# ahoynodnarb/minidiff

Measured on AMD Instinct MI355X. Metric: forward+backward passes/sec on 4096x4096 fp32 matmul+elementwise graph, higher is better.
Workload: dtype f32

## Files before the change

minidiff_amd/csrc/gemm.hip:

```cpp
#include <stdlib.h>

#include <algorithm>
#include <type_traits>
#include <utility>
#include <vector>

#include <hip/hip_ext.h>

#include "md_hip.h"

extern "C" int mdhip_alloc(size_t, void **);
extern "C" int mdhip_unary(int, const mdhip_array *, const mdhip_array *);
extern "C" int mdhip_free(void *);
extern "C" int mdhip_convert(const mdhip_array *, const mdhip_array *);

namespace {

typedef float f32x16 __attribute__((ext_vector_type(16)));
typedef float f32x4 __attribute__((ext_vector_type(4)));

constexpr int LDP = 4;

struct GemmArgs {
  const float *A, *B;
// ... 943 lines not shown
      if (s < 2) {
#pragma unroll
        for (int q = 0; q < 2; ++q) {
          glds64_krow(A, g.a_ks, kn * BK, CUR ? A0 : A1, (2 * s + q) * 4 + wave, lo);
          glds64_krow(B, g.b_ks, kn * BK, CUR ? B0 : B1, (2 * s + q) * 4 + wave, lo);
        }
      }
#pragma unroll
      for (int i = 0; i < WTM; ++i)
#pragma unroll
        for (int j = 0; j < WTN; ++j) acc[i][j] = __builtin_amdgcn_mfma_f64_16x16x4f64(fa[c][i], fb[c][j], acc[i][j], 0, 0, 0);
#pragma unroll
      for (int m = 0; m < WTM * WTN; ++m) {
        __builtin_amdgcn_sched_group_barrier(0x008, 1, 0);
        if (m < 8 && s + 1 < 4) __builtin_amdgcn_sched_group_barrier(0x100, 1, 0);
        if (s < 2 && m < 4) __builtin_amdgcn_sched_group_barrier(0x010, 1, 0);
      }
    }
    __syncthreads();
    MD_F64_READ(CUR ^ 1, 0, 0)
  };
  MD_KTILE_ROTATE(2, nk, ktile)
#undef MD_F64_READ
  MD_STORE_C64(false, acc, C, g, m0, n0, wm, wn, l16, h)
}


static const float *md_zero_block() {
  static const float *z = [] {
    void *p = nullptr;
    if (hipMalloc(&p, 64) != hipSuccess || hipMemset(p, 0, 64) != hipSuccess) return (const float *)nullptr;
    return (const float *)p;
  }();
  return z;
}

static bool md_gemm_nbuf3(int64_t blocks, int64_t K, int bk) {
  if (K < 2 * bk) return false;
  if (const int64_t f = md_opt(MD_OPT_GEMM_NBUF)) return f == 3;
  return blocks <= MD_NUM_CUS;
}

static void md_gemm_launch(void (*kernel)(GemmArgs), dim3 grid, int threads, const GemmArgs &ga) {
  hipEvent_t e0, e1;
  if (md_prof_take(&e0, &e1)) hipExtLaunchKernelGGL(kernel, grid, dim3((unsigned)threads), 0, md_stream(), e0, e1, 0, ga);
  else hipLaunchKernelGGL(kernel, grid, dim3((unsigned)threads), 0, md_stream(), ga);
}

struct StampDump {
  static constexpr size_t kMax = 8192;
  unsigned long long *dev = nullptr;
  int bm = 0, bn = 0, bk = 0;
  size_t blocks = 0;
  static StampDump &get() { static StampDump d; return d; }
  unsigned long long *buffer() {
    if (!dev) (void)hipMalloc((void **)&dev, kMax * 16);
    return dev;
  }
  void note(int m, int n, int k, size_t b) { bm = m; bn = n; bk = k; blocks = b; }
  ~StampDump() {
    if (!dev || !blocks) return;
    std::vector<unsigned long long> h(blocks * 2);
    if (hipDeviceSynchronize() != hipSuccess || hipMemcpy(h.data(), dev, h.size() * 8, hipMemcpyDeviceToHost) != hipSuccess) return;
    std::vector<double> ghz, us;
    for (size_t b = 0; b < blocks; ++b)
      if (h[2 * b + 1]) { ghz.push_back((double)h[2 * b] / (double)h[2 * b + 1] * 0.1); us.push_back((double)h[2 * b + 1] * 0.01); }
    std::sort(ghz.begin(), ghz.end());
    std::sort(us.begin(), us.end());
    if (!ghz.empty())
      fprintf(stderr, "[mdhip] last gemm %dx%dx%d: in-kernel clock median %.3f GHz (min %.3f, max %.3f) over %zu blocks; block main loop median %.1f us (min %.1f, p10 %.1f, p90 %.1f, max %.1f)\n",
              bm, bn, bk, ghz[ghz.size() / 2], ghz.front(), ghz.back(), ghz.size(), us[us.size() / 2], us.front(), us[us.size() / 10], us[us.size() * 9 / 10], us.back());
  }
};

enum { CFG_128x128x16 = 0, CFG_64x64x16, CFG_128x64x16, CFG_256x128x16, CFG_256x256x32, CFG_128x128x32, CFG_128x64x32, CFG_128x128_W8, CFG_COUNT };
struct Tile { int bm, bn, bk, wm, wn; };
struct TileCfg { Tile reg[2], dma[2]; double tf[2], tf_dma[2]; };
constexpr TileCfg kTiles[CFG_COUNT] = {
     {{{128, 128, 16, 2, 2}, {128, 128, 16, 2, 2}}, {{128, 128, 32, 2, 2}, {}}, {133.0, 0.0}, {143.0, 0.0}},
     {{{64, 64, 16, 2, 2}, {64, 64, 16, 2, 2}}, {{}, {}}, {120.0, 120.0}, {0.0, 0.0}},
     {{{128, 64, 16, 2, 2}, {128, 64, 16, 2, 2}}, {{}, {}}, {126.0, 0.0}, {0.0, 0.0}},
     {{{256, 128, 16, 2, 2}, {256, 128, 16, 2, 2}}, {{}, {}}, {139.0, 138.0}, {0.0, 0.0}},
     {{{256, 128, 16, 2, 2}, {256, 256, 32, 2, 2}}, {{256, 256, 32, 2, 2}, {256, 256, 32, 2, 2}}, {0.0, 140.0}, {149.0, 150.0}},
     {{{128, 128, 16, 2, 2}, {128, 128, 32, 2, 2}}, {{128, 128, 32, 2, 2}, {128, 128, 32, 2, 2}}, {0.0, 132.0}, {0.0, 146.0}},
     {{{128, 64, 16, 2, 2}, {128, 64, 32, 2, 2}}, {{}, {128, 64, 32, 2, 2}}, {0.0, 126.7}, {0.0, 138.0}},
     {{{128, 128, 16, 2, 4}, {128, 128, 32, 2, 4}}, {{128, 128, 32, 2, 4}, {128, 128, 32, 2, 4}}, {133.0, 134.0}, {143.5, 146.0}},
};
constexpr int kPickOrder[] = {CFG_256x256x32, CFG_256x128x16, CFG_128x128x16, CFG_128x128x32, CFG_128x128_W8, CFG_128x64x16, CFG_128x64x32, CFG_64x64x16};
constexpr bool lds3_fits(Tile t) { return 3 * (t.bm + t.bn) * t.bk * 4 <= 128 * 1024; }

static int pick_cfg(int64_t M, int64_t N, int64_t K, int64_t batch, bool tn, bool dma_ok, double *est = nullptr) {
  if (est) *est = 64.0 * 64.0 / 120.0;
  {
    const int64_t v = md_opt(MD_OPT_GEMM_CFG);
    if (v >= 0 && v < CFG_COUNT) return (int)v;
  }
  if (((M + 63) / 64) * ((N + 63) / 64) * batch < MD_NUM_CUS && K >= 1024) return CFG_64x64x16;
  int best = CFG_64x64x16;
  double best_t = 1e300;
  for (const int cfg : kPickOrder) {
    const TileCfg &c = kTiles[cfg];
    const bool dma = dma_ok && c.tf_dma[tn] > 0.0;
    const double tf = dma ? c.tf_dma[tn] : c.tf[tn];
    if (tf <= 0.0) continue;
    const Tile t = dma ? c.dma[tn] : c.reg[tn];
    const int64_t tiles = ((M + t.bm - 1) / t.bm) * ((N + t.bn - 1) / t.bn) * batch;
    double s = (double)((tiles + MD_NUM_CUS - 1) / MD_NUM_CUS) * t.bm * t.bn / tf;
    if (tiles <= MD_NUM_CUS && cfg != CFG_128x128_W8 && cfg != CFG_256x256x32 && !(tn && dma && cfg == CFG_128x128x32)) s /= 0.8;
    if (cfg == CFG_256x256x32 && tiles < MD_NUM_CUS) continue;
    if (!dma && ((M % t.bm) || (N % t.bn) || (K % 16))) s /= 0.85;
    if (s < best_t * 0.999) { best_t = s; best = cfg; }
  }
  if (est && best_t < 1e299) *est = best_t;
  return best;
}

template <class GA> static bool dma_family(const GA &ga, bool a_kc, bool b_kc) {
  return md_opt(MD_OPT_GEMM_GLDS) != 0 && (a_kc ? ga.a_ks == 1 : ga.a_ms == 1) && (b_kc ? ga.b_ks == 1 : ga.b_ns == 1) && (a_kc || !b_kc);
}
static bool dma_pieces_whole(const GemmArgs &ga, bool a_kc, bool b_kc) {
  return ((a_kc || b_kc) ? ga.K % 4 == 0 : true) && (a_kc || ga.M % 4 == 0 || ga.pad_m) && (b_kc || ga.N % 4 == 0 || ga.pad_n);
}
constexpr int64_t kLane32 = 1ll << 26;
template <class GA> static bool dma_strides(const GA &ga, bool a_kc, bool b_kc, int64_t lim) {
// ... 386 lines not shown
  constexpr bool TN = !A_KC && !B_KC;
  constexpr Tile R = kTiles[CFG].reg[TN], D = kTiles[CFG].dma[TN];
  constexpr int SCHED = R.bm == 64 ? 0 : 1;
  if (s.staging != ST_REG) {
    if constexpr (D.bm != 0 && A_KC) return kc_kernel<D.bm, D.bn, D.bk, D.wm, D.wn, B_KC>(s);
    else if constexpr (D.bm != 0 && TN) return tn_kernel<D.bm, D.bn, D.bk, D.wm, D.wn>(s);
    else return nullptr;
  }
  if (s.splits > 1) {
    if constexpr (R.bm == 64 && R.bn == 64) return s.edge ? k_gemm_f32_mfma<64, 64, 16, 2, 2, A_KC, B_KC, true, true> : k_gemm_f32_mfma<64, 64, 16, 2, 2, A_KC, B_KC, false, true>;
    else return nullptr;
  }
  if (s.epi) { if constexpr (A_KC && !B_KC) return k_gemm_f32_mfma<R.bm, R.bn, R.bk, R.wm, R.wn, true, false, false, false, SCHED, 1>; else return nullptr; }
  return s.edge ? k_gemm_f32_mfma<R.bm, R.bn, R.bk, R.wm, R.wn, A_KC, B_KC, true> : k_gemm_f32_mfma<R.bm, R.bn, R.bk, R.wm, R.wn, A_KC, B_KC, false, false, SCHED>;
}
template <bool A_KC, bool B_KC, int... C> static GemmKernel f32_kernel(const GemmStep &s, std::integer_sequence<int, C...>) {
  GemmKernel k = nullptr;
  ((s.cfg == C ? (void)(k = cfg_kernel<C, A_KC, B_KC>(s)) : (void)0), ...);
  return k;
}
static GemmKernel f32_kernel(const GemmStep &s) {
  return with_layout(s.a_kc, s.b_kc, [&](auto a, auto b) { return f32_kernel<decltype(a)::value, decltype(b)::value>(s, std::make_integer_sequence<int, CFG_COUNT>{}); });
}
static int run_step(const GemmStep &s, const void *const *tmp, int *skip) {
  auto at = [&](auto q) {
    const uintptr_t u = (uintptr_t)q;
    return (u >> 56) ? (decltype(q))((char *)tmp[(u >> 56) - 1] + (u & ((1ull << 56) - 1))) : q;
  };
  MdGemm g = s.g;
  g.a = at(g.a); g.b = at(g.b); g.c = at(g.c);
  switch (s.kind) {
    case S_LONGK:
    case S_SKINNY: {
      const int rc = s.kind == S_LONGK ? md_gemm_longk(g, s.dtype) : md_gemm_skinny(g, s.dtype);
      *skip = rc < 0 ? 0 : s.skip;
      return rc < 0 ? MDHIP_OK : rc;
    }
    case S_REPACK: {
      if (g.M <= 65535 * 4) {
        k_repack_rows<<<dim3((unsigned)((g.N + 1023) / 1024), (unsigned)((g.M + 3) / 4)), 256, 0, md_stream()>>>((const float *)g.a, g.M, g.N, g.a_ms, (float *)g.c, g.c_ms);
        return MD_LAUNCH_CHECK(s.what);
      }
      mdhip_array sd{}, dd{};
      sd.data = const_cast<void *>(g.a); sd.dtype = MDHIP_F32; sd.ndim = 2; sd.shape[0] = g.M; sd.shape[1] = g.N; sd.strides[0] = g.a_ms; sd.strides[1] = 1;
      dd = sd; dd.data = g.c; dd.strides[0] = g.c_ms;
      return mdhip_unary(MDHIP_U_COPY, &sd, &dd);
    }
    case S_F32: {
      GemmArgs ga = s.ga;
      ga.A = at(ga.A); ga.B = at(ga.B); ga.C = at(ga.C); ga.partial = at(ga.partial); ga.run_if_set = at(ga.run_if_set);
      if (s.epi) ga.tickets = md_tickets();
      const GemmKernel k = f32_kernel(s);
      if (!k) return md_fail(MDHIP_ERUNTIME, "matmul: no kernel for the planned launch (cfg %d)", s.cfg);
      if (s.stamp) ga.stamp = StampDump::get().buffer();
      if (s.stamp) StampDump::get().note(s.tile.bm, s.tile.bn, s.tile.bk, (size_t)s.grid.x * s.grid.z);
      if (s.splits > 1) hipLaunchKernelGGL(k, s.grid, dim3(64u * s.tile.wm * s.tile.wn), 0, md_stream(), ga);
      else md_gemm_launch(k, s.grid, 64 * s.tile.wm * s.tile.wn, ga);
      return MD_LAUNCH_CHECK(s.what);
    }
    case S_SUM:
      k_gemm_splitk_sum<<<md_grid_for(g.batch * g.M * g.N), MD_BLOCK, 0, md_stream()>>>((const float *)g.a, (int)g.K, g.batch, g.M, g.N, (float *)g.c,
                                                                                         g.c_bs, g.c_ms, g.c_ns);
      return MD_LAUNCH_CHECK(s.what);
    case S_F64: {
      auto k = with_layout(s.a_kc, s.b_kc, [&](auto a, auto b) -> void (*)(GemmArgs64) {
        constexpr bool A = decltype(a)::value, B = decltype(b)::value;
        if (s.cfg == 1) return s.edge ? k_gemm_f64_mfma<128, 128, 16, 2, 2, A, B, true> : k_gemm_f64_mfma<128, 128, 16, 2, 2, A, B, false>;
        return s.edge ? k_gemm_f64_mfma<64, 64, 16, 2, 2, A, B, true> : k_gemm_f64_mfma<64, 64, 16, 2, 2, A, B, false>;
      });
      hipLaunchKernelGGL(s.cfg == 2 ? k_gemm_f64_tn_glds : k, s.grid, dim3(256), 0, md_stream(), s.ga64);
      return MD_LAUNCH_CHECK(s.cfg == 2 ? "matmul(f64 mfma, direct-to-LDS)" : s.what);
    }
    case S_NMFMA: {
      const void *zero = s.edge ? md_zero_block() : nullptr;
      if (s.edge && !zero) return md_fail(MDHIP_EMEMORY, "matmul: zero block");
      return s.wide ? md_gemm_widen_mfma(g, s.dtype, s.a_kc, s.b_kc, s.edge, zero) : md_gemm_narrow_mfma(g, s.dtype, s.a_kc, s.b_kc, s.edge, zero);
    }
    case S_BX_CLEAR: return md_hip_check(hipMemsetAsync(const_cast<void *>(g.b), 0, 4, md_stream()), s.what);
    case S_BX_SPLIT_ROWS:
    case S_BX_SPLIT_COLS:
      return md_gemm_bf16x3_split((const float *)g.a, s.kind == S_BX_SPLIT_ROWS, g.M, g.K, g.a_ms, g.c, (unsigned *)const_cast<void *>(g.b), s.cfg,
                                  s.splits == 6 ? 3 : s.splits == 3 ? 2 : 1);
    case S_BX_GEMM:
      return md_gemm_bf16x3(g.a, at(s.b_planes), (float *)g.c, g.M, g.N, g.K, g.c_ms, (const unsigned *)g.b, (int)md_opt(MD_OPT_GEMM_BF16X3_LOOP), s.cfg,
                            (int)md_opt(MD_OPT_GEMM_BF16X3_BAND), s.splits);
    case S_NGENERIC: return s.wide ? md_gemm_widen_generic(g, s.dtype) : md_gemm_narrow_generic(g, s.dtype);
    case S_NCONV: {
      mdhip_array sd{}, dd{};
      sd.data = const_cast<void *>(g.a); sd.dtype = s.dtype; sd.ndim = 3;
      sd.shape[0] = g.batch; sd.shape[1] = g.M; sd.shape[2] = g.N;
      sd.strides[0] = g.a_bs; sd.strides[1] = g.a_ms; sd.strides[2] = g.a_ks;
      dd = sd; dd.data = g.c; dd.dtype = s.dtype_to;
      dd.strides[0] = g.c_bs; dd.strides[1] = g.c_ms; dd.strides[2] = g.c_ns;
      return mdhip_convert(&sd, &dd);
    }
    case S_GENERIC: {
      const dim3 grid((unsigned)((g.N + 15) / 16), (unsigned)((g.M + 15) / 16), (unsigned)g.batch);
      if (grid.y > 65535) return md_fail(MDHIP_EVALUE, "matmul: M too large for the generic kernel");
      switch (s.dtype) {
        case MDHIP_F32: k_gemm_generic<float><<<grid, 256, 0, md_stream()>>>(g); break;
        case MDHIP_F64: k_gemm_generic<double><<<grid, 256, 0, md_stream()>>>(g); break;
        case MDHIP_I32: k_gemm_generic<int32_t><<<grid, 256, 0, md_stream()>>>(g); break;
        default: k_gemm_generic<int64_t><<<grid, 256, 0, md_stream()>>>(g); break;
      }
      return MD_LAUNCH_CHECK(s.what);
    }
  }
  return md_fail(MDHIP_ERUNTIME, "matmul: unknown plan step");
}
static int run_plan(const GemmPlan &p) {
  void *tmp[GemmPlan::kMaxTmp] = {};
  int rc = MDHIP_OK;
  for (int i = 0; i < p.n && rc == MDHIP_OK; ++i) {
    for (int t = 0; t < p.ntmp && rc == MDHIP_OK; ++t) if (p.tmp[t].first == i) rc = mdhip_alloc(p.tmp[t].bytes, &tmp[t]);
    int skip = 0;
    if (rc == MDHIP_OK) rc = run_step(p.step[i], tmp, &skip);
    for (int t = 0; t < p.ntmp; ++t) if (p.tmp[t].last == i && tmp[t]) { mdhip_free(tmp[t]); tmp[t] = nullptr; }
    i += skip;
  }
  for (int t = 0; t < p.ntmp; ++t) if (tmp[t]) mdhip_free(tmp[t]);
  return rc;
}
struct HipExec {
  template <class Plan> static int run(const MdGemm &g, Plan &&plan) {
    if (g.batch > 65535) return md_fail(MDHIP_EVALUE, "matmul: batch extent %lld exceeds 65535", (long long)g.batch);
    GemmPlan p; plan(p);
    return run_plan(p);
  }
  template <class T> static int gemm(const MdGemm &g) { return run(g, [&](GemmPlan &p) { plan_gemm(p, g, md_dtype_of<T>::value); }); }
  static int gemm_narrow(const MdGemm &g, int dtype) { return run(g, [&](GemmPlan &p) { plan_narrow(p, g, dtype, false); }); }
  static int gemm_widen(const MdGemm &g, int dtype) { return run(g, [&](GemmPlan &p) { plan_narrow(p, g, dtype, true); }); }
};
static bool plan_epi(GemmPlan &p, GemmArgs ga) {
  bool plain_kc;
  {
    MdGemm g{1, ga.M, ga.N, ga.K, ga.A, ga.B, ga.C, 0, ga.a_ms, ga.a_ks, 0, ga.b_ks, ga.b_ns, 0, ga.c_ms, ga.c_ns};
    GemmPlan q;
    if (md_longk_shape(g) || plan_kranges(q, g)) return false;
// ... 65 lines not shown
```

minidiff_amd/csrc/gemm_bf16x3.hip:

```cpp
#include "md_hip.h"
#include "md_bf16x3.h"
#include "md_bf16x3_layout.h"

namespace {

typedef __attribute__((address_space(3))) void bx_lds_void;
typedef __attribute__((address_space(1))) const void bx_gbl_void;
typedef __bf16 bx_bf16x8 __attribute__((ext_vector_type(8)));
typedef int bx_i32x4 __attribute__((ext_vector_type(4)));
typedef float bx_f32x4 __attribute__((ext_vector_type(4)));
typedef float bx_f32x16 __attribute__((ext_vector_type(16)));

constexpr int BX_BM = 256, BX_BN = 128, BX_BK = 32;
constexpr int BX_NT = 512;
constexpr int BX_ROWB = BX_BK * 2;

__device__ __forceinline__ bool bx_split8(const float (&x)[8], bx_i32x4 *q1, bx_i32x4 *q2, bx_i32x4 *q3) {
  bool bad = false;
  uint32_t h[3][8];
#pragma unroll
  for (int j = 0; j < 8; ++j) {
    uint32_t p1, p2, p3;
    bad |= md_bf16x3_split(x[j], &p1, &p2, &p3);
    h[0][j] = p1 >> 16; h[1][j] = p2 >> 16; h[2][j] = p3 >> 16;
// ... 107 lines not shown
}

template <int NP>
__global__ void __launch_bounds__(256) k_bf16xp_split_rows_kt(const float *__restrict__ src, int64_t rows, int64_t K, int64_t rs, char *__restrict__ dst,
                                                              int64_t plane, unsigned *flag) {
  bool bad = false;
  const int l = threadIdx.x & 63, w = threadIdx.x >> 6;
  const int64_t k = (((int64_t)blockIdx.x * 4 + w) * 8 + (l >> 3)) * 32 + (l & 3) * 8;
  if (k < K) {
    for (int64_t r = (int64_t)blockIdx.y * 2 + ((l >> 2) & 1); r < rows; r += (int64_t)gridDim.y * 2) {
      const bx_f32x4 lo = *(const bx_f32x4 *)(src + r * rs + k), hi = *(const bx_f32x4 *)(src + r * rs + k + 4);
      const float x[8] = {lo[0], lo[1], lo[2], lo[3], hi[0], hi[1], hi[2], hi[3]};
      bx_i32x4 q[NP];
      bad |= bxp_split8<NP>(x, q);
      bxp_put<NP>(dst + md_bf16x3_plane_off(r, k, 64, rows * 64), plane, q);
    }
  }
  if (__syncthreads_or(bad) && threadIdx.x == 0) atomicOr(flag, 1u);
}

template <int NP>
__global__ void __launch_bounds__(256) k_bf16xp_split_cols(const float *__restrict__ src, int64_t rows, int64_t K, int64_t ks, char *__restrict__ dst,
                                                           int64_t plane, int64_t prs, int64_t pks, unsigned *flag) {
  __shared__ float T[32][66];
  const int t = threadIdx.x;
  for (int64_t kb = blockIdx.y; kb < K / 32; kb += gridDim.y) {
    const int64_t r0 = (int64_t)blockIdx.x * 64, k0 = kb * 32;
#pragma unroll
    for (int i = 0; i < 2; ++i) {
      const int idx = t + 256 * i, kk = idx >> 4, r4 = (idx & 15) * 4;
      const bx_f32x4 v = *(const bx_f32x4 *)(src + (k0 + kk) * ks + r0 + r4);
      T[kk][r4] = v[0]; T[kk][r4 + 1] = v[1]; T[kk][r4 + 2] = v[2]; T[kk][r4 + 3] = v[3];
    }
    __syncthreads();
    const int kg = t & 3, r = t >> 2;
    float x[8];
#pragma unroll
    for (int j = 0; j < 8; ++j) x[j] = T[kg * 8 + j][r];
    bx_i32x4 q[NP];
    const bool bad = bxp_split8<NP>(x, q);
    bxp_put<NP>(dst + md_bf16x3_plane_off(r0 + r, k0 + kg * 8, prs, pks), plane, q);
    if (__syncthreads_or(bad) && t == 0) atomicOr(flag, 1u);
  }
}

struct Bx3Args {
  const char *A, *B;
  float *C;
  int64_t K, c_ms;
  int64_t a_plane, b_plane;
  int64_t rs, a_kstep, b_kstep;
  int tiles_m, tiles_n, gm;
  const unsigned *flag;
};

__device__ __forceinline__ const char *bx_uniform(const char *p) {
  uint32_t lo = (uint32_t)(uintptr_t)p, hi = (uint32_t)((uintptr_t)p >> 32);
  asm("" : "+s"(lo), "+s"(hi));
  return reinterpret_cast<const char *>(((uintptr_t)hi << 32) | lo);
}

__device__ __forceinline__ void bx_piece(const char *P, int64_t rs, int64_t row, int64_t kstep, int kt, uint32_t lane_off, char *S) {
  uint32_t off = lane_off;
  asm("" : "+v"(off) : "s"(kt));
  const char *src = bx_uniform(P + row * rs + kt * kstep) + off;
  __builtin_amdgcn_global_load_lds((bx_gbl_void *)src, (bx_lds_void *)S, 16, 0, 0);
}

struct Bx3Bufs { char *a[3], *b[3]; };

template <int NP>
__device__ __forceinline__ void bx_stage(const Bx3Args &g, int64_t m0, int64_t n0, int kt, const Bx3Bufs &S, uint32_t lane_off) {
  const int wave = __builtin_amdgcn_readfirstlane(threadIdx.x >> 6);
#pragma unroll
  for (int p = 0; p < NP; ++p) {
#pragma unroll
    for (int i = 0; i < 2; ++i) bx_piece(g.A + p * g.a_plane, g.rs, m0 + 16 * (wave + 8 * i), g.a_kstep, kt, lane_off, S.a[p] + (wave + 8 * i) * 1024);
    bx_piece(g.B + p * g.b_plane, g.rs, n0 + 16 * wave, g.b_kstep, kt, lane_off, S.b[p] + wave * 1024);
  }
}

__device__ __forceinline__ bx_bf16x8 bx_frag(const char *S, int rb, int s) {
  const int l = threadIdx.x & 63, r = rb + (l & 31), c = 2 * s + (l >> 5);
  return __builtin_bit_cast(bx_bf16x8, *(const bx_i32x4 *)(S + r * BX_ROWB + ((c ^ ((r >> 2) & 3)) << 4)));
}

__device__ __forceinline__ bx_bf16x8 bx_frag_at(const char *S, uint32_t off, int half) {
  return __builtin_bit_cast(bx_bf16x8, *(const bx_i32x4 *)(S + off + half * 32 * BX_ROWB));
}
__device__ __forceinline__ uint32_t bx_read_off(int rb, int s) {
  const int l = threadIdx.x & 63, r = rb + (l & 31), c = 2 * s + (l >> 5);
  return (uint32_t)(r * BX_ROWB + ((c ^ ((r >> 2) & 3)) << 4));
}

template <int NP, int NPROD>
__device__ __forceinline__ void bx_mma(const Bx3Bufs &S, int wm, int wn, bx_f32x16 (&acc)[2][2]) {
  bx_f32x16 part[2][2];
#pragma unroll
  for (int i = 0; i < 2; ++i)
#pragma unroll
    for (int j = 0; j < 2; ++j)
#pragma unroll
      for (int e = 0; e < 16; ++e) part[i][j][e] = 0;
#pragma unroll
  for (int s = 0; s < 2; ++s) {
    bx_bf16x8 a[NP][2], b[NP][2];
// ... 48 lines not shown
  constexpr int PA[6] = {0, 0, 1, 0, 1, 2}, PB[6] = {0, 1, 0, 2, 1, 0};
  bx_f32x16 part[2][2];
  bx_bf16x8 a0[3][2], b0[3][2], a1[3][2], b1[3][2];
  uint32_t ra0 = rd[0], ra1 = rd[1], rb0 = rd[2], rb1 = rd[3];
  asm volatile("" : "+v"(ra0), "+v"(ra1), "+v"(rb0), "+v"(rb1));
  a0[0][0] = bx_frag_at(S.a[0], ra0, 0); b0[0][0] = bx_frag_at(S.b[0], rb0, 0); b0[0][1] = bx_frag_at(S.b[0], rb0, 1); a0[0][1] = bx_frag_at(S.a[0], ra0, 1);
  b0[1][0] = bx_frag_at(S.b[1], rb0, 0); b0[1][1] = bx_frag_at(S.b[1], rb0, 1);
  a0[1][0] = bx_frag_at(S.a[1], ra0, 0); a0[1][1] = bx_frag_at(S.a[1], ra0, 1);
  b0[2][0] = bx_frag_at(S.b[2], rb0, 0); b0[2][1] = bx_frag_at(S.b[2], rb0, 1);
  a0[2][0] = bx_frag_at(S.a[2], ra0, 0); a0[2][1] = bx_frag_at(S.a[2], ra0, 1);
  bx_fence();
#pragma unroll
  for (int q = 0; q < 6; ++q)
#pragma unroll
    for (int i = 0; i < 2; ++i)
#pragma unroll
      for (int j = 0; j < 2; ++j) {
        const int n = q * 4 + i * 2 + j;
        if (q == 0) {
          const bx_f32x16 zero = {0, 0, 0, 0, 0, 0, 0, 0, 0, 0, 0, 0, 0, 0, 0, 0};
          part[i][j] = __builtin_amdgcn_mfma_f32_32x32x16_bf16(a0[0][i], b0[0][j], zero, 0, 0, 0);
        } else {
          part[i][j] = __builtin_amdgcn_mfma_f32_32x32x16_bf16(a0[PA[q]][i], b0[PB[q]][j], part[i][j], 0, 0, 0);
        }
        if (n < 4) bx_fold4(acc[1][1], carry, 4 * n);
        if (n >= 4 && n <= 12) {
          if (STAGE) bx_dma_n(src, dst, n - 4, ka, kb, lane_off);
          if (n == 12) __builtin_amdgcn_s_waitcnt(0xC07F);
        }
        switch (n) {
          case 12: a1[0][0] = bx_frag_at(S.a[0], ra1, 0); b1[0][0] = bx_frag_at(S.b[0], rb1, 0); break;
          case 13: b1[1][0] = bx_frag_at(S.b[1], rb1, 0); a1[1][0] = bx_frag_at(S.a[1], ra1, 0); break;
          case 14: b1[2][0] = bx_frag_at(S.b[2], rb1, 0); a1[2][0] = bx_frag_at(S.a[2], ra1, 0); break;
          case 15: b1[0][1] = bx_frag_at(S.b[0], rb1, 1); b1[1][1] = bx_frag_at(S.b[1], rb1, 1); break;
          case 16: b1[2][1] = bx_frag_at(S.b[2], rb1, 1); a1[0][1] = bx_frag_at(S.a[0], ra1, 1); break;
          case 17: a1[1][1] = bx_frag_at(S.a[1], ra1, 1); a1[2][1] = bx_frag_at(S.a[2], ra1, 1); break;
          default: break;
        }
        bx_fence();
      }
#pragma unroll
  for (int t = 0; t < 4; ++t) {
    const int i = t >> 1, j = t & 1;
#pragma unroll
    for (int q = 0; q < 6; ++q) {
      part[i][j] = __builtin_amdgcn_mfma_f32_32x32x16_bf16(a1[PA[q]][i], b1[PB[q]][j], part[i][j], 0, 0, 0);
      if (t > 0 && q >= 2) bx_fold4(acc[(t - 1) >> 1][(t - 1) & 1], part[(t - 1) >> 1][(t - 1) & 1], 4 * (q - 2));
      bx_fence();
    }
  }
  carry = part[1][1];
}

__device__ __forceinline__ void bx_origin(const Bx3Args &g, int64_t *m0, int64_t *n0) {
  const int nwg = g.tiles_m * g.tiles_n, bid = blockIdx.x, xcd = bid & 7, q = nwg >> 3, r = nwg & 7;
  const int wg = (xcd < r ? xcd * (q + 1) : r * (q + 1) + (xcd - r) * q) + (bid >> 3);
  int tm, tn;
  md_bf16x3_tile(wg, g.tiles_m, g.tiles_n, g.gm, &tm, &tn);
  *m0 = (int64_t)tm * BX_BM; *n0 = (int64_t)tn * BX_BN;
}
__device__ __forceinline__ void bx_write_c(const Bx3Args &g, int64_t m0, int64_t n0, int wm, int wn, int l, const bx_f32x16 (&acc)[2][2]) {
#pragma unroll
  for (int i = 0; i < 2; ++i)
#pragma unroll
    for (int j = 0; j < 2; ++j)
#pragma unroll
      for (int e = 0; e < 16; ++e) {
        const int64_t m = m0 + wm * 64 + i * 32 + (e & 3) + 8 * (e >> 2) + 4 * (l >> 5), n = n0 + wn * 64 + j * 32 + (l & 31);
        g.C[m * g.c_ms + n] = acc[i][j][e];
      }
}

template <int LOOP>
__global__ void __launch_bounds__(BX_NT) k_gemm_bf16x3(Bx3Args g) {
  __shared__ __attribute__((aligned(16))) char sA00[BX_BM * BX_ROWB];
  __shared__ __attribute__((aligned(16))) char sA01[BX_BM * BX_ROWB];
  __shared__ __attribute__((aligned(16))) char sA02[BX_BM * BX_ROWB];
  __shared__ __attribute__((aligned(16))) char sB00[BX_BN * BX_ROWB];
  __shared__ __attribute__((aligned(16))) char sB01[BX_BN * BX_ROWB];
  __shared__ __attribute__((aligned(16))) char sB02[BX_BN * BX_ROWB];
  __shared__ __attribute__((aligned(16))) char sA10[BX_BM * BX_ROWB];
  __shared__ __attribute__((aligned(16))) char sA11[BX_BM * BX_ROWB];
  __shared__ __attribute__((aligned(16))) char sA12[BX_BM * BX_ROWB];
  __shared__ __attribute__((aligned(16))) char sB10[BX_BN * BX_ROWB];
  __shared__ __attribute__((aligned(16))) char sB11[BX_BN * BX_ROWB];
  __shared__ __attribute__((aligned(16))) char sB12[BX_BN * BX_ROWB];
  if (g.flag && *g.flag != 0) return;
  const Bx3Bufs S0{{sA00, sA01, sA02}, {sB00, sB01, sB02}}, S1{{sA10, sA11, sA12}, {sB10, sB11, sB12}};
  const int nwg = g.tiles_m * g.tiles_n, bid = blockIdx.x, xcd = bid & 7, q = nwg >> 3, r = nwg & 7;
  const int wg = (xcd < r ? xcd * (q + 1) : r * (q + 1) + (xcd - r) * q) + (bid >> 3);
  int tm, tn;
  md_bf16x3_tile(wg, g.tiles_m, g.tiles_n, g.gm, &tm, &tn);
  const int64_t m0 = (int64_t)tm * BX_BM, n0 = (int64_t)tn * BX_BN;
  const int wave = threadIdx.x >> 6, wm = wave >> 1, wn = wave & 1, l = threadIdx.x & 63;
  const int nk = (int)(g.K / BX_BK);
  const uint32_t lane_off = (uint32_t)((l >> 2) * g.rs + (((l & 3) ^ ((l >> 4) & 3)) << 4));
  bx_f32x16 acc[2][2];
#pragma unroll
  for (int i = 0; i < 2; ++i)
#pragma unroll
    for (int j = 0; j < 2; ++j)
#pragma unroll
      for (int e = 0; e < 16; ++e) acc[i][j][e] = 0;
  if constexpr (LOOP == 0) {
    bx_stage<3>(g, m0, n0, 0, S0, lane_off);
    for (int kt = 0; kt < nk; kt += 2) {
      __syncthreads();
      if (kt + 1 < nk) bx_stage<3>(g, m0, n0, kt + 1, S1, lane_off);
      bx_mma<3, 6>(S0, wm, wn, acc);
      if (kt + 1 >= nk) break;
      __syncthreads();
      if (kt + 2 < nk) bx_stage<3>(g, m0, n0, kt + 2, S0, lane_off);
      bx_mma<3, 6>(S1, wm, wn, acc);
    }
  } else {
    const int uw = __builtin_amdgcn_readfirstlane(wave);
    const int64_t rs = g.rs, ka = g.a_kstep, kb = g.b_kstep;
    Bx3Src src;
    Bx3Dst d0, d1;
#pragma unroll
    for (int p = 0; p < 3; ++p) {
#pragma unroll
      for (int i = 0; i < 2; ++i) {
        src.a[p][i] = bx_uniform(g.A + p * g.a_plane + (m0 + 16 * (uw + 8 * i)) * rs);
        d0.a[p][i] = S0.a[p] + (uw + 8 * i) * 1024;
        d1.a[p][i] = S1.a[p] + (uw + 8 * i) * 1024;
      }
      src.b[p] = bx_uniform(g.B + p * g.b_plane + (n0 + 16 * uw) * rs);
      d0.b[p] = S0.b[p] + uw * 1024;
      d1.b[p] = S1.b[p] + uw * 1024;
    }
    const uint32_t rd[4] = {bx_read_off(wm * 64, 0), bx_read_off(wm * 64, 1), bx_read_off(wn * 64, 0), bx_read_off(wn * 64, 1)};
    bx_f32x16 carry = {0, 0, 0, 0, 0, 0, 0, 0, 0, 0, 0, 0, 0, 0, 0, 0};
#pragma unroll
    for (int n = 0; n < 9; ++n) bx_dma_n(src, d0, n, 0, 0, lane_off);
    int kt = 0;
    for (; kt + 2 < nk; kt += 2) {
      __syncthreads();
      bx_tile<true>(S0, src, d1, ka, kb, lane_off, rd, acc, carry);
      __syncthreads();
      bx_tile<true>(S1, src, d0, ka, kb, lane_off, rd, acc, carry);
    }
    __syncthreads();
    if (kt + 1 < nk) {
      bx_tile<true>(S0, src, d1, ka, kb, lane_off, rd, acc, carry);
      __syncthreads();
      bx_tile<false>(S1, src, d0, 0, 0, lane_off, rd, acc, carry);
    } else {
      bx_tile<false>(S0, src, d1, 0, 0, lane_off, rd, acc, carry);
    }
#pragma unroll
    for (int e = 0; e < 16; e += 4) bx_fold4(acc[1][1], carry, e);
  }
#pragma unroll
  for (int i = 0; i < 2; ++i)
#pragma unroll
    for (int j = 0; j < 2; ++j)
#pragma unroll
      for (int e = 0; e < 16; ++e) {
        const int64_t m = m0 + wm * 64 + i * 32 + (e & 3) + 8 * (e >> 2) + 4 * (l >> 5), n = n0 + wn * 64 + j * 32 + (l & 31);
        g.C[m * g.c_ms + n] = acc[i][j][e];
      }
}

template <int NPROD>
__global__ void __launch_bounds__(BX_NT) k_gemm_bf16xp(Bx3Args g) {
  constexpr int NP = NPROD == 1 ? 1 : 2;
  __shared__ __attribute__((aligned(16))) char sA0[NP * BX_BM * BX_ROWB];
  __shared__ __attribute__((aligned(16))) char sB0[NP * BX_BN * BX_ROWB];
  __shared__ __attribute__((aligned(16))) char sA1[NP * BX_BM * BX_ROWB];
  __shared__ __attribute__((aligned(16))) char sB1[NP * BX_BN * BX_ROWB];
  if (g.flag && *g.flag != 0) return;
  const Bx3Bufs S0{{sA0, sA0 + (NP - 1) * BX_BM * BX_ROWB, nullptr}, {sB0, sB0 + (NP - 1) * BX_BN * BX_ROWB, nullptr}};
  const Bx3Bufs S1{{sA1, sA1 + (NP - 1) * BX_BM * BX_ROWB, nullptr}, {sB1, sB1 + (NP - 1) * BX_BN * BX_ROWB, nullptr}};
  int64_t m0, n0;
  bx_origin(g, &m0, &n0);
  const int wave = threadIdx.x >> 6, wm = wave >> 1, wn = wave & 1, l = threadIdx.x & 63;
  const int nk = (int)(g.K / BX_BK);
  const uint32_t lane_off = (uint32_t)((l >> 2) * g.rs + (((l & 3) ^ ((l >> 4) & 3)) << 4));
  bx_f32x16 acc[2][2];
#pragma unroll
  for (int i = 0; i < 2; ++i)
#pragma unroll
    for (int j = 0; j < 2; ++j)
#pragma unroll
      for (int e = 0; e < 16; ++e) acc[i][j][e] = 0;
  bx_stage<NP>(g, m0, n0, 0, S0, lane_off);
  for (int kt = 0; kt < nk; kt += 2) {
    __syncthreads();
    if (kt + 1 < nk) bx_stage<NP>(g, m0, n0, kt + 1, S1, lane_off);
    bx_mma<NP, NPROD>(S0, wm, wn, acc);
    if (kt + 1 >= nk) break;
    __syncthreads();
    if (kt + 2 < nk) bx_stage<NP>(g, m0, n0, kt + 2, S0, lane_off);
    bx_mma<NP, NPROD>(S1, wm, wn, acc);
  }
  bx_write_c(g, m0, n0, wm, wn, l, acc);
}

}

int md_gemm_bf16x3_split(const float *src, bool k_contig, int64_t rows, int64_t K, int64_t stride, void *planes, unsigned *flag, int layout, int nplanes) {
  const int64_t plane = rows * K * 2;
  char *dst = (char *)planes;
  if (k_contig && layout) {
    const dim3 grid((unsigned)((K / 32 + 31) / 32), (unsigned)(rows / 2 < 65535 ? rows / 2 : 65535));
    switch (nplanes) {
      case 1: k_bf16xp_split_rows_kt<1><<<grid, 256, 0, md_stream()>>>(src, rows, K, stride, dst, plane, flag); break;
      case 2: k_bf16xp_split_rows_kt<2><<<grid, 256, 0, md_stream()>>>(src, rows, K, stride, dst, plane, flag); break;
      default: k_bf16x3_split_rows_kt<<<grid, 256, 0, md_stream()>>>(src, rows, K, stride, dst, plane, flag); break;
    }
  } else if (k_contig) {
    const dim3 grid((unsigned)((K / 8 + 255) / 256), (unsigned)(rows < 65535 ? rows : 65535));
    switch (nplanes) {
      case 1: k_bf16xp_split_rows<1><<<grid, 256, 0, md_stream()>>>(src, rows, K, stride, dst, plane, flag); break;
      case 2: k_bf16xp_split_rows<2><<<grid, 256, 0, md_stream()>>>(src, rows, K, stride, dst, plane, flag); break;
      default: k_bf16x3_split_rows<<<grid, 256, 0, md_stream()>>>(src, rows, K, stride, dst, plane, flag); break;
    }
  } else {
    const dim3 grid((unsigned)(rows / 64), (unsigned)(K / 32 < 65535 ? K / 32 : 65535));
    const int64_t prs = md_bf16x3_row_stride(layout, K), pks = md_bf16x3_k_step(layout, rows);
    switch (nplanes) {
      case 1: k_bf16xp_split_cols<1><<<grid, 256, 0, md_stream()>>>(src, rows, K, stride, dst, plane, prs, pks, flag); break;
      case 2: k_bf16xp_split_cols<2><<<grid, 256, 0, md_stream()>>>(src, rows, K, stride, dst, plane, prs, pks, flag); break;
      default: k_bf16x3_split_cols<<<grid, 256, 0, md_stream()>>>(src, rows, K, stride, dst, plane, prs, pks, flag); break;
    }
  }
  return MD_LAUNCH_CHECK("matmul(bf16x3 split)");
}

int md_gemm_bf16x3(const void *a_planes, const void *b_planes, float *c, int64_t M, int64_t N, int64_t K, int64_t c_ms, const unsigned *flag, int loop,
                   int layout, int band, int products) {
  Bx3Args a{};
  a.A = (const char *)a_planes; a.B = (const char *)b_planes; a.C = c;
  a.K = K; a.c_ms = c_ms;
  a.a_plane = M * K * 2; a.b_plane = N * K * 2;
  a.rs = md_bf16x3_row_stride(layout, K); a.a_kstep = md_bf16x3_k_step(layout, M); a.b_kstep = md_bf16x3_k_step(layout, N);
  a.tiles_m = (int)(M / BX_BM); a.tiles_n = (int)(N / BX_BN);
  a.gm = md_bf16x3_band(a.tiles_m, MD_NUM_CUS / 8, band);
  a.flag = flag;
  md_opt_table()[MD_OPT_GEMM_BF16X3_RUNS] += 1;
  const dim3 grid((unsigned)(a.tiles_m * a.tiles_n));
  if (products == 1) MD_LAUNCH(k_gemm_bf16xp<1>, grid, BX_NT, a);
  else if (products == 3) MD_LAUNCH(k_gemm_bf16xp<3>, grid, BX_NT, a);
  else if (loop == 0) MD_LAUNCH(k_gemm_bf16x3<0>, grid, BX_NT, a);
  else MD_LAUNCH(k_gemm_bf16x3<1>, grid, BX_NT, a);
  return MD_LAUNCH_CHECK("matmul(f32 as bf16x3)");
}
```

minidiff_amd/csrc/md_hip.h:

```cpp
#pragma once
#include <hip/hip_runtime.h>
#include <hip/hip_ext.h>
#include <stdlib.h>

#include "md_dispatch.h"

#include "md_ticket.h"

hipStream_t md_stream();
struct MdGemm;
int md_gemm_skinny(const MdGemm &g, int dtype);
int md_gemm_longk(const MdGemm &g, int dtype);
int md_gemm_narrow_mfma(const MdGemm &g, int dtype, bool a_kc, bool b_kc, bool edge, const void *zero);
int md_gemm_narrow_generic(const MdGemm &g, int dtype);
int md_gemm_widen_mfma(const MdGemm &g, int dtype, bool a_kc, bool b_kc, bool edge, const void *zero);
int md_gemm_widen_generic(const MdGemm &g, int dtype);
int md_gemm_bf16x3_split(const float *src, bool k_contig, int64_t rows, int64_t K, int64_t stride, void *planes, unsigned *flag, int layout, int nplanes);
int md_gemm_bf16x3(const void *a_planes, const void *b_planes, float *c, int64_t M, int64_t N, int64_t K, int64_t c_ms, const unsigned *flag, int loop,
                   int layout, int band, int products);
unsigned *md_tickets();
bool md_capturing();
int *md_sticky();
int md_sticky_check();
bool md_prof_take(hipEvent_t *start, hipEvent_t *stop);
int md_hip_check(hipError_t e, const char *what);

#define MD_LAUNCH_CHECK(name) md_hip_check(hipGetLastError(), name)

#define MD_LAUNCH(kernel, grid, block, ...)                                                                            \
  do {                                                                                                                 \
    hipEvent_t md_e0_, md_e1_;                                                                                         \
    if (md_prof_take(&md_e0_, &md_e1_)) hipExtLaunchKernelGGL(kernel, dim3(grid), dim3(block), 0, md_stream(), md_e0_, md_e1_, 0, __VA_ARGS__); \
    else hipLaunchKernelGGL(kernel, dim3(grid), dim3(block), 0, md_stream(), __VA_ARGS__);                             \
  } while (0)

constexpr int MD_NUM_CUS = 256;
constexpr int MD_BLOCK = 256;
static inline int md_max_blocks() {
  const int n = (int)md_opt(MD_OPT_MAX_BLOCKS);
  return n > 0 ? n : MD_NUM_CUS * 8;
}
static inline int md_grid_for(int64_t work_items, int per_block = MD_BLOCK, int max_blocks = 0) {
  if (max_blocks <= 0) max_blocks = md_max_blocks();
  int64_t b = (work_items + per_block - 1) / per_block;
  if (b < 1) b = 1;
  if (b > max_blocks) b = max_blocks;
  return (int)b;
}

template <class T, int N> struct alignas(sizeof(T) * N > 16 ? 16 : sizeof(T) * N) MdVec {
  T v[N];
};

template <class T> __device__ __forceinline__ T md_shfl_down(T v, int delta) {
  if constexpr (sizeof(T) == 8) {
    union { T t; int32_t w[2]; } u;
    u.t = v;
    u.w[0] = __shfl_down(u.w[0], delta, 64);
    u.w[1] = __shfl_down(u.w[1], delta, 64);
    return u.t;
  } else if constexpr (sizeof(T) == 4) {
    union { T t; int32_t w; } u;
    u.t = v;
    u.w = __shfl_down(u.w, delta, 64);
    return u.t;
  } else {
    int32_t w = (int32_t)v;
    w = __shfl_down(w, delta, 64);
    return (T)w;
  }
}
```

minidiff_amd/csrc/md_options.h:

```cpp
#pragma once
#include <stdint.h>
#include <stdlib.h>
#include <string.h>

#define MD_OPTION_LIST(X)                                                                                                        \
                                                                                    \
  X(PINNED_CAP, "pinned_cap", (int64_t)4 << 30, 'c')                  \
  X(JIT, "jit", 1, 'c')                                      \
  X(JIT_VERBOSE, "jit_verbose", 0, 'c')                                           \
  X(INDEX_DEFER, "index_defer", 0, 'c')                 \
                                                              \
  X(JIT_MIN, "jit_min", 1 << 18, 'x')                                   \
  X(COMM_PRIORITY, "comm_priority", 0, 'x')                         \
  X(MAX_BLOCKS, "max_blocks", 0, 'x')                                      \
  X(NT, "nt", -1, 'x')                                      \
  X(GEMM_CFG, "gemm_cfg", -1, 'x')                                  \
  X(GEMM_GLDS, "gemm_glds", 1, 'x')                                                   \
  X(GEMM_NBUF, "gemm_nbuf", 0, 'x')                     \
  X(GEMM_PEEL, "gemm_peel", 1, 'x')                            \
  X(GEMM_TT_SWAP, "gemm_tt_swap", 1, 'x')                                \
  X(GEMM_REPACK, "gemm_repack", 1, 'x')                         \
  X(GEMM_SUPER, "gemm_super", 8, 'x')                                      \
  X(GEMM_SPLITK, "gemm_splitk", 1, 'x')                                                                                         \
  X(GEMM_STAMP, "gemm_stamp", 0, 'x')                                                  \
  X(GEMM_F64_MFMA, "gemm_f64_mfma", 1, 'x')                                                                                     \
  X(GEMM_SKINNY, "gemm_skinny", 1, 'x')                                \
  X(GEMM_WIDEN, "gemm_widen", 1, 'x')                   \
  X(GEMM_BF16X3, "gemm_bf16x3", 1, 'x')                 \
  X(GEMM_BF16X3_RUNS, "gemm_bf16x3_runs", 0, 'x')       \
  X(GEMM_BF16X3_LOOP, "gemm_bf16x3_loop", 1, 'x')       \
  X(GEMM_BF16X3_BAND, "gemm_bf16x3_band", 0, 'x')       \
  X(GEMM_BF16X3_PLANES, "gemm_bf16x3_planes", 1, 'x')   \
  X(GEMM_PRODUCTS, "gemm_products", 6, 'x')             \
  X(JIT_U, "jit_u", 0, 'x')                             \
  X(JIT_BLOCKS, "jit_blocks", 0, 'x')                                       \
  X(JIT_AXES_WIDE, "jit_axes_wide", 0, 'x')             \
  X(SWEEP_NB, "sweep_nb", 0, 'x')                                         \
  X(SWEEP_RU, "sweep_ru", 0, 'x')                                                                                               \
  X(SWEEP_NT_STORE, "sweep_nt_store", 1, 'x')                                                                                   \
  X(ROWS_WAVE, "rows_wave", 1, 'x')                                                                                             \
  X(COLS_NB, "cols_nb", 0, 'x')                                                                                                 \
  X(ROWS_BLOCKS, "rows_blocks", 0, 'x')                                          \
  X(ARG_BLOCKS, "arg_blocks", 0, 'x')                                   \
  X(ARG_BATCHED, "arg_batched", 1, 'x')                 \
  X(VAR_BATCHED, "var_batched", 1, 'x')                      \
  X(GATHER_RUNS, "gather_runs", 1, 'x')                                                                                         \
  X(SCATTER_CENSUS, "scatter_census", 1, 'x')                                                                                   \
  X(SCATTER_SORTED, "scatter_sorted", 1, 'x')

enum MdOptId {
#define MD_OPT_ENUM(ID, name, dflt, kind) MD_OPT_##ID,
  MD_OPTION_LIST(MD_OPT_ENUM)
#undef MD_OPT_ENUM
  MD_OPT_COUNT
};

struct MdOptDef {
  const char *name;
  int64_t dflt;
  char kind;
};

inline const MdOptDef *md_opt_defs() {
  static const MdOptDef defs[MD_OPT_COUNT] = {
#define MD_OPT_DEF(ID, name, dflt, kind) {name, (int64_t)(dflt), kind},
      MD_OPTION_LIST(MD_OPT_DEF)
#undef MD_OPT_DEF
  };
  return defs;
}

inline int64_t *md_opt_table() {
  static int64_t table[MD_OPT_COUNT];
  static const bool loaded = [] {
    const MdOptDef *d = md_opt_defs();
    const char *ex = getenv("MDHIP_EXPERIMENTS");
    const bool experiments = ex && ex[0] == '1' && ex[1] == 0;
    for (int i = 0; i < MD_OPT_COUNT; ++i) {
      table[i] = d[i].dflt;
      if (d[i].kind == 'x' && !experiments) continue;
      char env[64] = "MDHIP_";
      size_t n = strlen(env);
      for (const char *p = d[i].name; *p && n + 1 < sizeof env; ++p) env[n++] = (char)((*p >= 'a' && *p <= 'z') ? *p - 32 : *p);
// ... 16 lines not shown
```

Measured before the change: 559.6.

## Add ping-pong bf16x3 main loop with split-wave barriers and make it default

Adds a new LOOP==2 main loop for the bf16x3 GEMM. Its waves are offset by a barrier so the two halves alternate between the LDS-read/DMA phase and the MFMA phase. Each tile accumulates the six bf16 products into per-fragment partials that are folded into the fp32 accumulators once per tile, instead of using a single carry. It becomes the default loop variant and is meant to overlap memory traffic with matrix-core work better. The change also adds optional per-block cycle stamping for the bf16x3 kernel, which reports cycles per k-tile. The extra barriers and partial registers add register pressure and synchronization risk.

```diff
diff --git a/minidiff_amd/csrc/gemm.hip b/minidiff_amd/csrc/gemm.hip
--- a/minidiff_amd/csrc/gemm.hip
+++ b/minidiff_amd/csrc/gemm.hip
@@ -1019,24 +1019,29 @@
   unsigned long long *dev = nullptr;
   int bm = 0, bn = 0, bk = 0;
   size_t blocks = 0;
+  int64_t ktiles = 0;
   static StampDump &get() { static StampDump d; return d; }
   unsigned long long *buffer() {
     if (!dev) (void)hipMalloc((void **)&dev, kMax * 16);
     return dev;
   }
-  void note(int m, int n, int k, size_t b) { bm = m; bn = n; bk = k; blocks = b; }
+  void note(int m, int n, int k, size_t b, int64_t kt = 0) { bm = m; bn = n; bk = k; blocks = b; ktiles = kt; }
   ~StampDump() {
     if (!dev || !blocks) return;
     std::vector<unsigned long long> h(blocks * 2);
     if (hipDeviceSynchronize() != hipSuccess || hipMemcpy(h.data(), dev, h.size() * 8, hipMemcpyDeviceToHost) != hipSuccess) return;
-    std::vector<double> ghz, us;
+    std::vector<double> ghz, us, cyc;
     for (size_t b = 0; b < blocks; ++b)
-      if (h[2 * b + 1]) { ghz.push_back((double)h[2 * b] / (double)h[2 * b + 1] * 0.1); us.push_back((double)h[2 * b + 1] * 0.01); }
+      if (h[2 * b + 1]) { ghz.push_back((double)h[2 * b] / (double)h[2 * b + 1] * 0.1); us.push_back((double)h[2 * b + 1] * 0.01); cyc.push_back((double)h[2 * b]); }
     std::sort(ghz.begin(), ghz.end());
     std::sort(us.begin(), us.end());
+    std::sort(cyc.begin(), cyc.end());
     if (!ghz.empty())
       fprintf(stderr, "[mdhip] last gemm %dx%dx%d: in-kernel clock median %.3f GHz (min %.3f, max %.3f) over %zu blocks; block main loop median %.1f us (min %.1f, p10 %.1f, p90 %.1f, max %.1f)\n",
               bm, bn, bk, ghz[ghz.size() / 2], ghz.front(), ghz.back(), ghz.size(), us[us.size() / 2], us.front(), us[us.size() / 10], us[us.size() * 9 / 10], us.back());
+    if (!cyc.empty() && ktiles > 0)
+      fprintf(stderr, "[mdhip] last gemm %dx%dx%d: %lld k-tiles per block, shader cycles per k-tile and CU median %.0f (min %.0f, p10 %.0f, p90 %.0f, max %.0f)\n", bm, bn, bk,
+              (long long)ktiles, cyc[cyc.size() / 2] / ktiles, cyc.front() / ktiles, cyc[cyc.size() / 10] / ktiles, cyc[cyc.size() * 9 / 10] / ktiles, cyc.back() / ktiles);
   }
 };
 
@@ -1529,8 +1534,9 @@
       if (s.epi) ga.tickets = md_tickets();
       const GemmKernel k = f32_kernel(s);
       if (!k) return md_fail(MDHIP_ERUNTIME, "matmul: no kernel for the planned launch (cfg %d)", s.cfg);
-      if (s.stamp) ga.stamp = StampDump::get().buffer();
-      if (s.stamp) StampDump::get().note(s.tile.bm, s.tile.bn, s.tile.bk, (size_t)s.grid.x * s.grid.z);
+      const bool stamped = s.stamp && !ga.run_if_set;
+      if (stamped) ga.stamp = StampDump::get().buffer();
+      if (stamped) StampDump::get().note(s.tile.bm, s.tile.bn, s.tile.bk, (size_t)s.grid.x * s.grid.z);
       if (s.splits > 1) hipLaunchKernelGGL(k, s.grid, dim3(64u * s.tile.wm * s.tile.wn), 0, md_stream(), ga);
       else md_gemm_launch(k, s.grid, 64 * s.tile.wm * s.tile.wn, ga);
       return MD_LAUNCH_CHECK(s.what);
@@ -1558,9 +1564,13 @@
     case S_BX_SPLIT_COLS:
       return md_gemm_bf16x3_split((const float *)g.a, s.kind == S_BX_SPLIT_ROWS, g.M, g.K, g.a_ms, g.c, (unsigned *)const_cast<void *>(g.b), s.cfg,
                                   s.splits == 6 ? 3 : s.splits == 3 ? 2 : 1);
-    case S_BX_GEMM:
+    case S_BX_GEMM: {
+      const int64_t tiles = (g.M / 256) * (g.N / 128);
+      unsigned long long *stamp = s.splits == 6 && md_gemm_stamped(tiles) ? StampDump::get().buffer() : nullptr;
+      if (stamp) StampDump::get().note(256, 128, 32, (size_t)tiles, g.K / 32);
       return md_gemm_bf16x3(g.a, at(s.b_planes), (float *)g.c, g.M, g.N, g.K, g.c_ms, (const unsigned *)g.b, (int)md_opt(MD_OPT_GEMM_BF16X3_LOOP), s.cfg,
-                            (int)md_opt(MD_OPT_GEMM_BF16X3_BAND), s.splits);
+                            (int)md_opt(MD_OPT_GEMM_BF16X3_BAND), s.splits, stamp);
+    }
     case S_NGENERIC: return s.wide ? md_gemm_widen_generic(g, s.dtype) : md_gemm_narrow_generic(g, s.dtype);
     case S_NCONV: {
       mdhip_array sd{}, dd{};
diff --git a/minidiff_amd/csrc/gemm_bf16x3.hip b/minidiff_amd/csrc/gemm_bf16x3.hip
--- a/minidiff_amd/csrc/gemm_bf16x3.hip
+++ b/minidiff_amd/csrc/gemm_bf16x3.hip
@@ -183,6 +183,7 @@
   int64_t rs, a_kstep, b_kstep;
   int tiles_m, tiles_n, gm;
   const unsigned *flag;
+  unsigned long long *stamp;
 };
 
 __device__ __forceinline__ const char *bx_uniform(const char *p) {
@@ -337,6 +338,65 @@
   carry = part[1][1];
 }
 
+__device__ __forceinline__ void bx2_barrier() {
+  bx_fence();
+  asm volatile("" ::: "memory");
+  __builtin_amdgcn_s_barrier();
+  asm volatile("" ::: "memory");
+  bx_fence();
+}
+
+template <bool STAGE>
+__device__ __forceinline__ void bx2_tile(const Bx3Bufs &S, Bx3Src &src, const Bx3Dst &dst, int64_t ka, int64_t kb, uint32_t lane_off, const uint32_t (&rd)[4],
+                                         bx_f32x16 (&acc)[2][2], bx_f32x16 (&part)[2][2]) {
+  constexpr int PA[6] = {0, 0, 1, 0, 1, 2}, PB[6] = {0, 1, 0, 2, 1, 0};
+  constexpr int NL = 3, CSTEP = 4;
+#pragma unroll
+  for (int s = 0; s < 2; ++s) {
+    bx_bf16x8 a[3][2], b[3][2];
+    uint32_t ra = rd[s], rb = rd[2 + s];
+    asm volatile("" : "+v"(ra), "+v"(rb));
+    a[0][0] = bx_frag_at(S.a[0], ra, 0); b[0][0] = bx_frag_at(S.b[0], rb, 0); b[0][1] = bx_frag_at(S.b[0], rb, 1); a[0][1] = bx_frag_at(S.a[0], ra, 1);
+    b[1][0] = bx_frag_at(S.b[1], rb, 0); b[1][1] = bx_frag_at(S.b[1], rb, 1);
+    a[1][0] = bx_frag_at(S.a[1], ra, 0); a[1][1] = bx_frag_at(S.a[1], ra, 1);
+    b[2][0] = bx_frag_at(S.b[2], rb, 0); b[2][1] = bx_frag_at(S.b[2], rb, 1);
+    a[2][0] = bx_frag_at(S.a[2], ra, 0); a[2][1] = bx_frag_at(S.a[2], ra, 1);
+    bx_fence();
+    if (s == 0) {
+      if (STAGE) {
+#pragma unroll
+        for (int n = 0; n < NL; ++n) bx_dma_n(src, dst, n, ka, kb, lane_off);
+      }
+      bx_fence();
+#pragma unroll
+      for (int t = 0; t < 4; ++t)
+#pragma unroll
+        for (int e = 0; e < 16; e += 4) bx_fold4(acc[t >> 1][t & 1], part[t >> 1][t & 1], e);
+      bx_fence();
+    }
+    if (s == 0) __builtin_amdgcn_s_waitcnt(0xC07F);
+    else __builtin_amdgcn_s_waitcnt(0x0070);
+    bx2_barrier();
+#pragma unroll
+    for (int q = 0; q < 6; ++q)
+#pragma unroll
+      for (int i = 0; i < 2; ++i)
+#pragma unroll
+        for (int j = 0; j < 2; ++j) {
+          const int n = q * 4 + i * 2 + j;
+          if (s == 0 && q == 0) {
+            const bx_f32x16 zero = {0, 0, 0, 0, 0, 0, 0, 0, 0, 0, 0, 0, 0, 0, 0, 0};
+            part[i][j] = __builtin_amdgcn_mfma_f32_32x32x16_bf16(a[0][i], b[0][j], zero, 0, 0, 0);
+          } else {
+            part[i][j] = __builtin_amdgcn_mfma_f32_32x32x16_bf16(a[PA[q]][i], b[PB[q]][j], part[i][j], 0, 0, 0);
+          }
+          if (STAGE && s == 0 && n % CSTEP == 1 && NL + n / CSTEP < 9) bx_dma_n(src, dst, NL + n / CSTEP, ka, kb, lane_off);
+          bx_fence();
+        }
+    bx2_barrier();
+  }
+}
+
 __device__ __forceinline__ void bx_origin(const Bx3Args &g, int64_t *m0, int64_t *n0) {
   const int nwg = g.tiles_m * g.tiles_n, bid = blockIdx.x, xcd = bid & 7, q = nwg >> 3, r = nwg & 7;
   const int wg = (xcd < r ? xcd * (q + 1) : r * (q + 1) + (xcd - r) * q) + (bid >> 3);
@@ -356,7 +416,7 @@
       }
 }
 
-template <int LOOP>
+template <int LOOP, bool STAMP = false>
 __global__ void __launch_bounds__(BX_NT) k_gemm_bf16x3(Bx3Args g) {
   __shared__ __attribute__((aligned(16))) char sA00[BX_BM * BX_ROWB];
   __shared__ __attribute__((aligned(16))) char sA01[BX_BM * BX_ROWB];
@@ -387,6 +447,11 @@
     for (int j = 0; j < 2; ++j)
 #pragma unroll
       for (int e = 0; e < 16; ++e) acc[i][j][e] = 0;
+  unsigned long long st_c = 0, st_r = 0;
+  if constexpr (STAMP) {
+    st_c = __builtin_amdgcn_s_memtime(); st_r = __builtin_amdgcn_s_memrealtime();
+    __builtin_amdgcn_s_waitcnt(0xC07F);
+  }
   if constexpr (LOOP == 0) {
     bx_stage<3>(g, m0, n0, 0, S0, lane_off);
     for (int kt = 0; kt < nk; kt += 2) {
@@ -416,26 +481,64 @@
       d1.b[p] = S1.b[p] + uw * 1024;
     }
     const uint32_t rd[4] = {bx_read_off(wm * 64, 0), bx_read_off(wm * 64, 1), bx_read_off(wn * 64, 0), bx_read_off(wn * 64, 1)};
-    bx_f32x16 carry = {0, 0, 0, 0, 0, 0, 0, 0, 0, 0, 0, 0, 0, 0, 0, 0};
-#pragma unroll
-    for (int n = 0; n < 9; ++n) bx_dma_n(src, d0, n, 0, 0, lane_off);
-    int kt = 0;
-    for (; kt + 2 < nk; kt += 2) {
+    if constexpr (LOOP == 1) {
+      bx_f32x16 carry = {0, 0, 0, 0, 0, 0, 0, 0, 0, 0, 0, 0, 0, 0, 0, 0};
+#pragma unroll
+      for (int n = 0; n < 9; ++n) bx_dma_n(src, d0, n, 0, 0, lane_off);
+      int kt = 0;
+      for (; kt + 2 < nk; kt += 2) {
+        __syncthreads();
+        bx_tile<true>(S0, src, d1, ka, kb, lane_off, rd, acc, carry);
+        __syncthreads();
+        bx_tile<true>(S1, src, d0, ka, kb, lane_off, rd, acc, carry);
+      }
       __syncthreads();
-      bx_tile<true>(S0, src, d1, ka, kb, lane_off, rd, acc, carry);
-      __syncthreads();
-      bx_tile<true>(S1, src, d0, ka, kb, lane_off, rd, acc, carry);
-    }
-    __syncthreads();
-    if (kt + 1 < nk) {
-      bx_tile<true>(S0, src, d1, ka, kb, lane_off, rd, acc, carry);
-      __syncthreads();
-      bx_tile<false>(S1, src, d0, 0, 0, lane_off, rd, acc, carry);
+      if (kt + 1 < nk) {
+        bx_tile<true>(S0, src, d1, ka, kb, lane_off, rd, acc, carry);
+        __syncthreads();
+        bx_tile<false>(S1, src, d0, 0, 0, lane_off, rd, acc, carry);
+      } else {
+        bx_tile<false>(S0, src, d1, 0, 0, lane_off, rd, acc, carry);
+      }
+#pragma unroll
+      for (int e = 0; e < 16; e += 4) bx_fold4(acc[1][1], carry, e);
     } else {
-      bx_tile<false>(S0, src, d1, 0, 0, lane_off, rd, acc, carry);
-    }
-#pragma unroll
-    for (int e = 0; e < 16; e += 4) bx_fold4(acc[1][1], carry, e);
+      const int half = uw >> 2;
+      bx_f32x16 part[2][2];
+#pragma unroll
+      for (int i = 0; i < 2; ++i)
+#pragma unroll
+        for (int j = 0; j < 2; ++j)
+#pragma unroll
+          for (int e = 0; e < 16; ++e) part[i][j][e] = 0;
+#pragma unroll
+      for (int n = 0; n < 9; ++n) bx_dma_n(src, d0, n, 0, 0, lane_off);
+      __builtin_amdgcn_s_waitcnt(0x0070);
+      bx2_barrier();
+      if (half) bx2_barrier();
+      int kt = 0;
+      for (; kt + 2 < nk; kt += 2) {
+        bx2_tile<true>(S0, src, d1, ka, kb, lane_off, rd, acc, part);
+        bx2_tile<true>(S1, src, d0, ka, kb, lane_off, rd, acc, part);
+      }
+      if (kt + 1 < nk) {
+        bx2_tile<true>(S0, src, d1, ka, kb, lane_off, rd, acc, part);
+        bx2_tile<false>(S1, src, d0, 0, 0, lane_off, rd, acc, part);
+      } else {
+        bx2_tile<false>(S0, src, d1, 0, 0, lane_off, rd, acc, part);
+      }
+#pragma unroll
+      for (int t = 0; t < 4; ++t)
+#pragma unroll
+        for (int e = 0; e < 16; e += 4) bx_fold4(acc[t >> 1][t & 1], part[t >> 1][t & 1], e);
+      if (!half) bx2_barrier();
+    }
+  }
+  if constexpr (STAMP) {
+    if (threadIdx.x == 0) {
+      g.stamp[2 * blockIdx.x] = __builtin_amdgcn_s_memtime() - st_c;
+      g.stamp[2 * blockIdx.x + 1] = __builtin_amdgcn_s_memrealtime() - st_r;
+    }
   }
 #pragma unroll
   for (int i = 0; i < 2; ++i)
@@ -515,7 +618,7 @@
 }
 
 int md_gemm_bf16x3(const void *a_planes, const void *b_planes, float *c, int64_t M, int64_t N, int64_t K, int64_t c_ms, const unsigned *flag, int loop,
-                   int layout, int band, int products) {
+                   int layout, int band, int products, unsigned long long *stamp) {
   Bx3Args a{};
   a.A = (const char *)a_planes; a.B = (const char *)b_planes; a.C = c;
   a.K = K; a.c_ms = c_ms;
@@ -524,11 +627,16 @@
   a.tiles_m = (int)(M / BX_BM); a.tiles_n = (int)(N / BX_BN);
   a.gm = md_bf16x3_band(a.tiles_m, MD_NUM_CUS / 8, band);
   a.flag = flag;
+  a.stamp = stamp;
   md_opt_table()[MD_OPT_GEMM_BF16X3_RUNS] += 1;
   const dim3 grid((unsigned)(a.tiles_m * a.tiles_n));
   if (products == 1) MD_LAUNCH(k_gemm_bf16xp<1>, grid, BX_NT, a);
   else if (products == 3) MD_LAUNCH(k_gemm_bf16xp<3>, grid, BX_NT, a);
+  else if (stamp && loop == 0) MD_LAUNCH((k_gemm_bf16x3<0, true>), grid, BX_NT, a);
+  else if (stamp && loop == 2) MD_LAUNCH((k_gemm_bf16x3<2, true>), grid, BX_NT, a);
+  else if (stamp) MD_LAUNCH((k_gemm_bf16x3<1, true>), grid, BX_NT, a);
   else if (loop == 0) MD_LAUNCH(k_gemm_bf16x3<0>, grid, BX_NT, a);
+  else if (loop == 2) MD_LAUNCH(k_gemm_bf16x3<2>, grid, BX_NT, a);
   else MD_LAUNCH(k_gemm_bf16x3<1>, grid, BX_NT, a);
   return MD_LAUNCH_CHECK("matmul(f32 as bf16x3)");
 }
diff --git a/minidiff_amd/csrc/md_hip.h b/minidiff_amd/csrc/md_hip.h
--- a/minidiff_amd/csrc/md_hip.h
+++ b/minidiff_amd/csrc/md_hip.h
@@ -17,7 +17,7 @@
 int md_gemm_widen_generic(const MdGemm &g, int dtype);
 int md_gemm_bf16x3_split(const float *src, bool k_contig, int64_t rows, int64_t K, int64_t stride, void *planes, unsigned *flag, int layout, int nplanes);
 int md_gemm_bf16x3(const void *a_planes, const void *b_planes, float *c, int64_t M, int64_t N, int64_t K, int64_t c_ms, const unsigned *flag, int loop,
-                   int layout, int band, int products);
+                   int layout, int band, int products, unsigned long long *stamp);
 unsigned *md_tickets();
 bool md_capturing();
 int *md_sticky();
diff --git a/minidiff_amd/csrc/md_options.h b/minidiff_amd/csrc/md_options.h
--- a/minidiff_amd/csrc/md_options.h
+++ b/minidiff_amd/csrc/md_options.h
@@ -28,7 +28,7 @@
   X(GEMM_WIDEN, "gemm_widen", 1, 'x')                   \
   X(GEMM_BF16X3, "gemm_bf16x3", 1, 'x')                 \
   X(GEMM_BF16X3_RUNS, "gemm_bf16x3_runs", 0, 'x')       \
-  X(GEMM_BF16X3_LOOP, "gemm_bf16x3_loop", 1, 'x')       \
+  X(GEMM_BF16X3_LOOP, "gemm_bf16x3_loop", 2, 'x')       \
   X(GEMM_BF16X3_BAND, "gemm_bf16x3_band", 0, 'x')       \
   X(GEMM_BF16X3_PLANES, "gemm_bf16x3_planes", 1, 'x')   \
   X(GEMM_PRODUCTS, "gemm_products", 6, 'x')             \
```

Result: faster. 592.6, median of 6 (+5.9%).
